# SCUT-CCNL/3DSIFT

Measured on AMD Instinct MI355X. Metric: Mvoxels/s end-to-end KpSiftAlgorithm on 512^3 fp32, higher is better.
Workload: dtype f32

## Files before the change

### 3dsift_amd/csrc/context.hip

```cpp
#include <float.h>
#include <math.h>
#include <stdlib.h>
#include <string.h>

#include <algorithm>
#include <atomic>
#include <mutex>
#include <thread>

#include "ctx_internal.h"

#pragma clang fp contract(off)

namespace s3d {

static thread_local std::string g_last_error;
void set_last_error(const std::string &s) { g_last_error = s; }

int set_device(int device) {
	int n = 0;
	if (hipGetDeviceCount(&n) != hipSuccess || n <= 0) {
		set_last_error("no HIP device visible: this library has no CPU fallback");
		return SIFT3D_ERR_NO_DEVICE;
	}
// ... 150 lines not shown
	c->gss.assign((size_t)c->noct * c->ng, Level());
	c->dog.assign((size_t)c->noct * c->nd, Level());
	for (int pyr = 0; pyr < 2; pyr++) {
		const int interval = pyr ? c->nd : c->ng;
		std::vector<Level> &P = pyr ? c->dog : c->gss;
		int nx = c->nx, ny = c->ny, nz = c->nz;
		float u = (float)(1 << c->octave_base);
		for (int o = 0; o < c->noct; o++) {
			for (int s = 0; s < interval; s++) {
				Level &L = P[(size_t)o * interval + s];
				L.nx = nx; L.ny = ny; L.nz = nz; L.unit = u;
				L.scale = level_scale(c->p, o + c->octave_base, s);
				if (c->slab) { L.bz = c->own1 - c->own0 + 2 * c->halo; L.zoff = c->own0 - c->halo; }
			}
			nx /= 2; ny /= 2; nz /= 2;
			u *= 2;
		}
	}
}

int upload_luts(sift3d_ctx *c, const std::vector<WinLut> &luts, std::vector<float> &pool) {
	if (pool.empty()) pool.push_back(-1.0f);
	if (c->d_luts) { S3D_HIP(hipFree(c->d_luts)); c->d_luts = nullptr; }
	if (c->d_lutpool) { S3D_HIP(hipFree(c->d_lutpool)); c->d_lutpool = nullptr; }
	S3D_HIP(hipMalloc(&c->d_luts, sizeof(WinLut) * luts.size()));
	S3D_HIP(hipMalloc(&c->d_lutpool, sizeof(float) * pool.size()));
	S3D_HIP(hipMemcpy(c->d_luts, luts.data(), sizeof(WinLut) * luts.size(), hipMemcpyHostToDevice));
	S3D_HIP(hipMemcpy(c->d_lutpool, pool.data(), sizeof(float) * pool.size(), hipMemcpyHostToDevice));
	return SIFT3D_OK;
}

std::vector<WinLut> blank_luts(const sift3d_ctx *c) {
	std::vector<WinLut> luts((size_t)std::max(1, c->noct + c->octave_base) * 8 * 2);
	for (auto &l : luts) { l.off = 0; l.len = 0; l.nin = -1; l.radius = 0; l.sigma = 0; l.fix_scale = 1.0f; l.wsum = 1.0f; l.list_off = -1; l.list_R = 0; }
	return luts;
}

static int build_luts(sift3d_ctx *c) {
	std::vector<WinLut> luts = blank_luts(c);
	std::vector<float> pool;
	for (int o = 0; o < c->noct; o++)
		for (int lv = 1; lv <= c->p.num_kp_levels && lv < 8; lv++) {
			const Level &D = c->dog[(size_t)o * c->nd + lv];
			const float u = D.unit, scale = D.scale;
			for (int which = 0; which < 2; which++) {
				float sigma, radius;
				if (which == 0) { sigma = 1.5f * scale; radius = sigma * 3.0f; }
				else { sigma = scale * 7.071067812f; radius = 2.0f * sigma; }
				if (!append_lut(pool, luts[((size_t)(o + c->octave_base) * 8 + lv) * 2 + which], which, sigma, radius, u, scale)) c->desc_lut_lds = false;
			}
		}
	return upload_luts(c, luts, pool);
}

static size_t al64(size_t n) { return (n + 63) & ~(size_t)63; }

size_t arena_floats_of(const sift3d_ctx *c) {
	size_t total = c->in_own ? 0 : al64(c->in.n());
	if (!c->slab) for (int o = 0; o < c->noct; o++) total += 2 * al64(c->gss[(size_t)o * c->ng].n());
	for (auto &L : c->gss) total += al64(L.n());
	for (auto &L : c->dog) total += al64(L.n());
	return total;
}

int create_common(sift3d_handle *out, const CreateCfg &cfg, const sift3d_params *params, int device) {
	*out = nullptr;
	if (cfg.nx <= 0 || cfg.ny <= 0 || cfg.nz <= 0) { set_last_error("bad dimensions"); return SIFT3D_ERR_ARG; }
// ... 785 lines not shown
```

### 3dsift_amd/csrc/kernels_orient.hip

```cpp
#include <float.h>

#include "sift3d_internal.h"

namespace s3d {

__device__ __forceinline__ float wave_sum(float v) {
#pragma unroll
	for (int o = 32; o > 0; o >>= 1) v = v + __shfl_xor(v, o, 64);
	return v;
}

__device__ __forceinline__ void win_bounds(float c, float rad, float u, int n, int &lo, int &hi) {
	int s = (int)floorf(c - __fdiv_rn(rad, u));
	lo = s > 1 ? s : 1;
	int e = (int)ceilf(c + __fdiv_rn(rad, u));
	hi = e < (n - 2) ? e : n - 2;
}

__device__ void eig_sym3(const double A[9], double w[3], double V[9]) {
	double a[9];
#pragma unroll
	for (int i = 0; i < 9; i++) { a[i] = A[i]; V[i] = (i % 4 == 0) ? 1.0 : 0.0; }
	for (int sweep = 0; sweep < 64; sweep++) {
		const double off = fabs(a[1]) + fabs(a[2]) + fabs(a[5]);
		const double diag = fabs(a[0]) + fabs(a[4]) + fabs(a[8]);
		if (off <= 1e-300 || off <= 1e-22 * diag) break;
#pragma unroll
		for (int pq = 0; pq < 3; pq++) {
			const int p = (pq == 2) ? 1 : 0, q = (pq == 0) ? 1 : 2;
			const double apq = a[3 * p + q];
			if (apq == 0.0) continue;
			const double theta = (a[4 * q] - a[4 * p]) / (2.0 * apq);
			const double t = (theta >= 0 ? 1.0 : -1.0) / (fabs(theta) + sqrt(theta * theta + 1.0));
// ... 71 lines not shown
	if ((double)fabsf(val[0] - val[1]) < DBL_EPSILON || (double)fabsf(val[0] - val[2]) < DBL_EPSILON ||
	    (double)fabsf(val[2] - val[1]) < DBL_EPSILON)
		return -2;

	const float d_norm = sqrtf(dot3f(w3, w3));
	float corner = FLT_MAX;
	for (int i = 2; i > 0; i--) {
		const float d = dot3f(vec[i], w3);
		const float q_norm = sqrtf(dot3f(vec[i], vec[i]));
		const float cos_ang = __fdiv_rn(d, d_norm * q_norm);
		const float a = fabsf(cos_ang);
		corner = corner < a ? corner : a;
		const float sgn = d > 0.0f ? 1.0f : -1.0f;
		vec[i][0] *= sgn; vec[i][1] *= sgn; vec[i][2] *= sgn;
	}
	nr = nr || fabsf(corner - corner_thresh) <= 1e-4f;
	if (near) *near = nr;
	if (corner < corner_thresh) return -3;
	if (near) *near = true;
	const float *v1 = vec[2], *v2 = vec[1];
	float vr[3];
	vr[0] = v1[1] * v2[2] - v1[2] * v2[1];
	vr[1] = v1[2] * v2[0] - v1[0] * v2[2];
	vr[2] = v1[0] * v2[1] - v1[1] * v2[0];
	kp.rot[0] = v1[0]; kp.rot[1] = v2[0]; kp.rot[2] = vr[0];
	kp.rot[3] = v1[1]; kp.rot[4] = v2[1]; kp.rot[5] = vr[1];
	kp.rot[6] = v1[2]; kp.rot[7] = v2[2]; kp.rot[8] = vr[2];
	return 1;
}

#ifndef S3D_ORI_UN
#define S3D_ORI_UN 2
#endif
constexpr int kTileW = 28, kTileH = 27;
constexpr int kTilePc = ((kTileW / 4) * kTileH + 63) / 64;
typedef float f4o __attribute__((ext_vector_type(4), aligned(4)));
constexpr int kOriLut = 256;

constexpr int kTermPitch = 68;
template <bool EXACT>
__global__ void __launch_bounds__(256) k_orient(DevKp *__restrict__ kps, int *__restrict__ codes, const unsigned *__restrict__ d_count, unsigned cap,
                                                const LevelRef *__restrict__ levels, const WinLut *__restrict__ luts,
                                                const float *__restrict__ lutpool, float max_eig, float corner, int part_rank,
                                                int part_world, const int *__restrict__ redo_list, const unsigned *__restrict__ redo_count) {
	__shared__ __attribute__((aligned(16))) float s_tile[4 * 3 * kTileW * kTileH];
	__shared__ float s_wlut[4 * kOriLut];
	__shared__ __attribute__((aligned(16))) float s_terms[EXACT ? 4 * 9 * kTermPitch : 4];
	const unsigned count = min(d_count[0], cap);
	const int lane = threadIdx.x & 63;
	const unsigned wave = blockIdx.x * (blockDim.x >> 6) + (threadIdx.x >> 6);
	const unsigned nwaves = gridDim.x * (blockDim.x >> 6);
	const unsigned pw = part_world > 1 ? (unsigned)part_world : 1u, pr = part_world > 1 ? (unsigned)part_rank : 0u;
	if (!EXACT && pw > 1)
		for (unsigned k = blockIdx.x * blockDim.x + threadIdx.x; k < count; k += gridDim.x * blockDim.x)
			if (k % pw != pr) { kps[k].code = 0; codes[k] = 0; }
	const unsigned owned = EXACT ? min(redo_count[0], cap) : (count > pr ? (count - pr + pw - 1) / pw : 0u);
	float *tb = &s_terms[EXACT ? (threadIdx.x >> 6) * 9 * kTermPitch : 0];
	for (unsigned j = wave; j < owned; j += nwaves) {
		const unsigned k = EXACT ? (unsigned)redo_list[j] : j * pw + pr;
		const int cxi = kps[k].x, cyi = kps[k].y, czi = kps[k].z;
		const int li = kps[k].octave * 8 + kps[k].level;
		const LevelRef L = levels[li];
		const WinLut lut = luts[li * 2 + 0];
		const float *__restrict__ wtab = lutpool + lut.off;
		const float u = L.unit, inv_u = __fdiv_rn(1.0f, u);
		int x0, x1, y0, y1, z0, z1;
		win_bounds((float)cxi, lut.radius, u, L.nx, x0, x1);
		win_bounds((float)cyi, lut.radius, u, L.ny, y0, y1);
		win_bounds((float)czi, lut.radius, u, L.nz, z0, z1);
		const int wx = x1 - x0 + 1, wy = y1 - y0 + 1;
		const int plane = (wx > 0 && wy > 0) ? wx * wy : 0;
		const float inv_wx = 1.0f / (float)(wx > 0 ? wx : 1);
		const size_t sy = (size_t)L.nx, sz = (size_t)L.nx * L.ny;
		const gfloat_p Ld = as_global(L.d);
		float t00 = 0.f, t01 = 0.f, t02 = 0.f, t11 = 0.f, t12 = 0.f, t22 = 0.f, g0 = 0.f, g1 = 0.f, g2 = 0.f;
		float chain = 0.f;
		auto emit = [&](bool ok, float c1p, float c1m, float c2p, float c2m, float c3p, float c3m, float ww, int nvalid) {
			float vx = 0.5f * (c1p - c1m);
			float vy = 0.5f * (c2p - c2m);
			float vz = 0.5f * (c3p - c3m);
			vx = vx * inv_u; vy = vy * inv_u; vz = vz * inv_u;
			if (!EXACT) {
				if (ok) {
					const float wx = vx * ww, wy = vy * ww, wz = vz * ww;
					t00 = __fmaf_rn(vx, wx, t00);
					t01 = __fmaf_rn(vx, wy, t01);
					t02 = __fmaf_rn(vx, wz, t02);
					t11 = __fmaf_rn(vy, wy, t11);
					t12 = __fmaf_rn(vy, wz, t12);
					t22 = __fmaf_rn(vz, wz, t22);
					g0 = g0 + wx; g1 = g1 + wy; g2 = g2 + wz;
				}
			} else {
				tb[0 * kTermPitch + lane] = ok ? vx * vx * ww : 0.0f;
				tb[1 * kTermPitch + lane] = ok ? vx * vy * ww : 0.0f;
				tb[2 * kTermPitch + lane] = ok ? vx * vz * ww : 0.0f;
				tb[3 * kTermPitch + lane] = ok ? vy * vy * ww : 0.0f;
				tb[4 * kTermPitch + lane] = ok ? vy * vz * ww : 0.0f;
				tb[5 * kTermPitch + lane] = ok ? vz * vz * ww : 0.0f;
				tb[6 * kTermPitch + lane] = ok ? vx * ww : 0.0f;
				tb[7 * kTermPitch + lane] = ok ? vy * ww : 0.0f;
				tb[8 * kTermPitch + lane] = ok ? vz * ww : 0.0f;
				__builtin_amdgcn_fence(__ATOMIC_RELEASE, "wavefront");
				__builtin_amdgcn_wave_barrier();
				__builtin_amdgcn_fence(__ATOMIC_ACQUIRE, "wavefront");
				if (lane < 9) {
					const float4 *row = reinterpret_cast<const float4 *>(tb + lane * kTermPitch);
#pragma unroll
					for (int h = 0; h < 2; h++) {
						if (h * 32 >= nvalid) break;
						float4 v[8];
#pragma unroll
						for (int i = 0; i < 8; i++) v[i] = row[h * 8 + i];
#pragma unroll
						for (int i = 0; i < 8; i++) { chain = chain + v[i].x; chain = chain + v[i].y; chain = chain + v[i].z; chain = chain + v[i].w; }
					}
				}
				__builtin_amdgcn_wave_barrier();
			}
		};
		const int tw = wx + 2, th = wy + 2;
		if (plane > 0 && z1 >= z0 && tw <= kTileW && th <= kTileH && lut.len <= kOriLut) {
			float *tile = &s_tile[(threadIdx.x >> 6) * 3 * kTileW * kTileH];
			float *wl = &s_wlut[(threadIdx.x >> 6) * kOriLut];
			for (int i = lane; i < lut.len && i < kOriLut; i += 64) wl[i] = wtab[i];
			const int npx = (tw + 3) >> 2;
			const int tnp = npx * th;
			const float inv_npx = 1.0f / (float)npx;
			int toff[kTilePc];
			int goff[kTilePc];
#pragma unroll
			for (int i = 0; i < kTilePc; i++) {
				const int idx = lane + 64 * i;
				const int ty = (int)(((float)idx + 0.5f) * inv_npx);
				const int px = idx - ty * npx;
				const bool ok = idx < tnp;
				toff[i] = ok ? ty * kTileW + 4 * px : -1;
				goff[i] = ok ? (x0 - 1 + 4 * px) + (int)sy * (y0 - 1 + ty) : (x0 - 1) + (int)sy * (y0 - 1);
			}
			const gfloat_p base = Ld - sz * (size_t)L.zoff;
			f4o pf[kTilePc];
			auto request = [&](int zp) {
				const gfloat_p pl = base + sz * (size_t)zp;
#pragma unroll
				for (int i = 0; i < kTilePc; i++) pf[i] = *reinterpret_cast<const f4o __attribute__((address_space(1))) *>(pl + goff[i]);
			};
			auto deposit = [&](int slot) {
				float *dstp = tile + slot * (kTileW * kTileH);
#pragma unroll
				for (int i = 0; i < kTilePc; i++)
					if (toff[i] >= 0) *reinterpret_cast<float4 *>(dstp + toff[i]) = make_float4(pf[i].x, pf[i].y, pf[i].z, pf[i].w);
			};
			request(z0 - 1); deposit(0);
			request(z0);     deposit(1);
			request(z0 + 1);
			int sm = 0, sc = 1, sp = 2;
			constexpr int kEL = 8;
			const unsigned *__restrict__ lst = reinterpret_cast<const unsigned *>(lutpool) + (lut.list_off >= 0 ? lut.list_off : 0);
			const int LR = lut.list_R;
			const unsigned *__restrict__ ent = lst + 2 * LR + 2;
			const bool use_list = lut.list_off >= 0 && (int)lst[LR + 1] - (int)lst[LR] <= 64 * kEL;
			const int ox = cxi - x0 - 128, oy = cyi - y0 - 128;
			unsigned En[kEL];
			int cntn = 0;
			auto fetch_entries = [&](int dzp) {
				const int pi = dzp + LR;
				const bool has = use_list && pi >= 0 && pi <= 2 * LR;
				const int e0 = has ? (int)lst[pi] : 0, e1 = has ? (int)lst[pi + 1] : 0;
				cntn = e1 - e0;
#pragma unroll
				for (int i = 0; i < kEL; i++) {
					const int idx = e0 + i * 64 + lane;
					En[i] = ent[idx < e1 ? idx : e0];
				}
			};
			fetch_entries(z0 - czi);
			for (int z = z0; z <= z1; z++) {
#if !defined(S3D_ODIAG) || !(S3D_ODIAG & 2)
				deposit(sp);
				request(min(z + 2, z1 + 1));
#endif
				__builtin_amdgcn_fence(__ATOMIC_RELEASE, "wavefront");
				__builtin_amdgcn_wave_barrier();
				__builtin_amdgcn_fence(__ATOMIC_ACQUIRE, "wavefront");
				const float *pm = tile + sm * (kTileW * kTileH), *pc = tile + sc * (kTileW * kTileH), *pp = tile + sp * (kTileW * kTileH);
				const int dz = z - czi;
				constexpr int kUn = S3D_ORI_UN;
#ifdef S3D_ODIAG
				if (S3D_ODIAG & 1) { } else
#endif
				if (use_list) {
					unsigned E[kEL];
#pragma unroll
					for (int i = 0; i < kEL; i++) E[i] = En[i];
					const int cnt = cntn;
					fetch_entries(dz + 1);
#pragma unroll
					for (int p0 = 0; p0 < kEL; p0 += kUn) {
						if (p0 * 64 >= cnt) break;
						float nb[kUn][6], w[kUn];
#pragma unroll
						for (int q = 0; q < kUn; q++) {
							const unsigned e = E[p0 + q];
							const int lx = (int)(e & 255u) + ox, ly = (int)((e >> 8) & 255u) + oy;
							const bool ok = (p0 + q) * 64 + lane < cnt && (unsigned)lx < (unsigned)wx && (unsigned)ly < (unsigned)wy;
							w[q] = ok ? wl[e >> 16] : -1.0f;
							const int o = ok ? __mul24(ly + 1, kTileW) + lx + 1 : kTileW + 1;
							nb[q][0] = pc[o + 1]; nb[q][1] = pc[o - 1]; nb[q][2] = pc[o + kTileW]; nb[q][3] = pc[o - kTileW];
							nb[q][4] = pp[o]; nb[q][5] = pm[o];
						}
#pragma unroll
						for (int q = 0; q < kUn; q++) {
							if (EXACT && (p0 + q) * 64 >= cnt) break;
							emit(!(w[q] < 0.0f), nb[q][0], nb[q][1], nb[q][2], nb[q][3], nb[q][4], nb[q][5], w[q], min(64, cnt - (p0 + q) * 64));
						}
					}
				} else if (EXACT) {
					for (int vb = 0; vb < plane; vb += 64) {
						const int v = vb + lane;
						const int ly = (int)(((float)v + 0.5f) * inv_wx);
						const int lx = v - ly * wx;
						const int dx = x0 + lx - cxi, dy = y0 + ly - cyi;
						const int n = dx * dx + dy * dy + dz * dz;
						const bool in = v < plane && n < lut.len;
						const float ww = in ? wl[n] : -1.0f;
						const int o = in ? __mul24(ly + 1, kTileW) + lx + 1 : kTileW + 1;
						emit(!(ww < 0.0f), pc[o + 1], pc[o - 1], pc[o + kTileW], pc[o - kTileW], pp[o], pm[o], ww, min(64, plane - vb));
					}
				} else
				for (int v0 = lane; v0 < plane; v0 += 64 * kUn) {
					float nb[kUn][6], w[kUn];
#pragma unroll
					for (int q = 0; q < kUn; q++) {
						const int v = v0 + 64 * q;
						const int ly = (int)(((float)v + 0.5f) * inv_wx);
						const int lx = v - ly * wx;
						const int dx = x0 + lx - cxi, dy = y0 + ly - cyi;
						const int n = dx * dx + dy * dy + dz * dz;
						const bool ok = v < plane && n < lut.len;
						w[q] = ok ? wl[n] : -1.0f;
						const int o = ok ? __mul24(ly + 1, kTileW) + lx + 1 : kTileW + 1;
						nb[q][0] = pc[o + 1]; nb[q][1] = pc[o - 1]; nb[q][2] = pc[o + kTileW]; nb[q][3] = pc[o - kTileW];
						nb[q][4] = pp[o]; nb[q][5] = pm[o];
					}
#pragma unroll
					for (int q = 0; q < kUn; q++)
						emit(!(w[q] < 0.0f), nb[q][0], nb[q][1], nb[q][2], nb[q][3], nb[q][4], nb[q][5], w[q], 64);
				}
				__builtin_amdgcn_wave_barrier();
				const int tmp = sm; sm = sc; sc = sp; sp = tmp;
			}
		} else
		for (int z = z0; z <= z1; z++) {
			const int dz = z - czi;
			for (int vb = 0; vb < plane; vb += 64) {
				const int v = vb + lane;
				const int ly = (int)(((float)v + 0.5f) * inv_wx);
				const int lx = v - ly * wx;
				const int x = x0 + lx, y = y0 + ly;
				const int dx = x - cxi, dy = y - cyi;
				const int n = dx * dx + dy * dy + dz * dz;
				const bool in = v < plane && n < lut.len;
				const float w = in ? wtab[n] : -1.0f;
				const bool ok = !(w < 0.0f);
				const gfloat_p c = ok ? Ld + (size_t)x + sy * (size_t)y + sz * (size_t)(z - L.zoff)
				                      : Ld + (size_t)cxi + sy * (size_t)cyi + sz * (size_t)(czi - L.zoff);
				emit(ok, c[1], c[-1], c[sy], *(c - sy), c[sz], *(c - sz), w, min(64, plane - vb));
			}
		}
// ... 9 lines not shown
			if (lane == 0) {
				kps[k].st[0] = T6[0]; kps[k].st[1] = T6[1]; kps[k].st[2] = T6[2]; kps[k].st[4] = T6[3]; kps[k].st[5] = T6[4]; kps[k].st[8] = T6[5];
				kps[k].win[0] = w3[0]; kps[k].win[1] = w3[1]; kps[k].win[2] = w3[2];
			}
		}
	}
}

__global__ void __launch_bounds__(64) k_orient_finish(DevKp *__restrict__ kps, int *__restrict__ codes, const unsigned *__restrict__ d_count,
                                                      unsigned cap, float max_eig, float corner, int part_rank, int part_world, int pass,
                                                      int *__restrict__ redo_list, unsigned *__restrict__ redo_count) {
	const unsigned count = min(d_count[0], cap);
	const unsigned pw = part_world > 1 ? (unsigned)part_world : 1u, pr = part_world > 1 ? (unsigned)part_rank : 0u;
	const unsigned owned = pass ? min(redo_count[0], cap) : (count > pr ? (count - pr + pw - 1) / pw : 0u);
	for (unsigned j = blockIdx.x * blockDim.x + threadIdx.x; j < owned; j += gridDim.x * blockDim.x) {
		const unsigned k = pass ? (unsigned)redo_list[j] : j * pw + pr;
		DevKp kp = kps[k];
		const float T6[6] = {kp.st[0], kp.st[1], kp.st[2], kp.st[4], kp.st[5], kp.st[8]};
		const float w3[3] = {kp.win[0], kp.win[1], kp.win[2]};
		bool near = false;
		kp.code = finish_orientation(kp, T6, w3, max_eig, corner, &near);
		kps[k] = kp;
		codes[k] = kp.code == 1 ? ((kp.level << 4) | 1) : kp.code;
		if (!pass && near) {
			const unsigned pos = atomicAdd(redo_count, 1u);
			if (pos < cap) redo_list[pos] = (int)k;
		}
	}
}

void launch_orient(DevKp *kps, int *codes, const unsigned *d_count, unsigned cap, const LevelRef *d_levels, const WinLut *d_luts,
                   const float *d_lutpool, float max_eig, float corner, int part_rank, int part_world, int *redo_list, unsigned *redo_count,
                   hipStream_t st) {
	static const int ori_grid = dev_tune_i("S3D_ORI_GRID", 256 * 32);
	(void)hipMemsetAsync(redo_count, 0, sizeof(unsigned), st);
	hipLaunchKernelGGL(k_orient<false>, dim3(ori_grid), dim3(256), 0, st, kps, codes, d_count, cap, d_levels, d_luts, d_lutpool, max_eig, corner,
	                   part_rank, part_world, (const int *)redo_list, (const unsigned *)redo_count);
	hipLaunchKernelGGL(k_orient_finish, dim3(256 * 8), dim3(64), 0, st, kps, codes, d_count, cap, max_eig, corner, part_rank, part_world, 0,
	                   redo_list, redo_count);
	hipLaunchKernelGGL(k_orient<true>, dim3(ori_grid), dim3(256), 0, st, kps, codes, d_count, cap, d_levels, d_luts, d_lutpool, max_eig, corner,
	                   part_rank, part_world, (const int *)redo_list, (const unsigned *)redo_count);
	hipLaunchKernelGGL(k_orient_finish, dim3(256 * 2), dim3(64), 0, st, kps, codes, d_count, cap, max_eig, corner, part_rank, part_world, 1,
	                   redo_list, redo_count);
}

static_assert(offsetof(DevKp, st) + sizeof(float) * 9 - offsetof(DevKp, win) == sizeof(float) * (kOrientWords - 1), "DevKp layout");

__global__ void __launch_bounds__(256) k_orient_pack(const DevKp *__restrict__ kps, const unsigned *__restrict__ d_count, unsigned cap,
                                                     int *__restrict__ dst, int part_rank, int part_world) {
	const unsigned count = min(d_count[0], cap);
	const unsigned total = count * (unsigned)kOrientWords;
	for (unsigned i = blockIdx.x * blockDim.x + threadIdx.x; i < total; i += gridDim.x * blockDim.x) {
		const unsigned k = i / kOrientWords, w = i - k * kOrientWords;
		int v = 0;
		if (part_world <= 1 || (int)(k % (unsigned)part_world) == part_rank)
			v = w == 0 ? kps[k].code : __float_as_int(kps[k].win[w - 1]);
		dst[i] = v;
	}
}

__global__ void __launch_bounds__(256) k_orient_unpack(DevKp *__restrict__ kps, int *__restrict__ codes, const unsigned *__restrict__ d_count,
                                                       unsigned cap, const int *__restrict__ src) {
	const unsigned count = min(d_count[0], cap);
	const unsigned total = count * (unsigned)kOrientWords;
	for (unsigned i = blockIdx.x * blockDim.x + threadIdx.x; i < total; i += gridDim.x * blockDim.x) {
		const unsigned k = i / kOrientWords, w = i - k * kOrientWords;
		const int v = src[i];
// ... 116 lines not shown
```

### 3dsift_amd/csrc/sift3d_internal.h

```cpp
#pragma once

#include <hip/hip_runtime.h>
#include <stdint.h>

#include <string>
#include <vector>

#include "../../include/sift3d_hip.h"
#include "../../include/sift3d_hip_test.h"

#pragma clang fp contract(off)

namespace s3d {

#ifndef S3D_MAX_HW
#define S3D_MAX_HW 64
#endif
constexpr int kMaxHW = S3D_MAX_HW;
constexpr int kMaxTaps = 2 * kMaxHW + 1;
constexpr int kDesc = SIFT3D_DESC_NUMEL;
constexpr int kFaces = 20;

struct Taps {
	int hw;
// ... 23 lines not shown
	size_t n() const { return (size_t)nx * ny * planes(); }
	ZRange zr(int zo0, int zo1) const { return ZRange{planes(), zoff, nz, zo0, zo1}; }
	ZRange zr_all() const { return ZRange{planes(), zoff, nz, 0, planes()}; }
};

struct DevKp {
	int x, y, z;
	int octave, level;
	float scale;
	int code;
	int slot;
	float win[3];
	float eigvalue[3];
	float eigvector[9];
	float rot[9];
	float st[9];
};

struct FaceConst {
	float e1[3], e2[3], t[3], q[3];
	float qe2;
	int idx[3];
	float centre[3];
};

struct WinLut {
	int off;
	int len;
	int nin;
	float radius;
	float sigma;
	float fix_scale;
	float wsum;
	int list_off, list_R;
};
constexpr int kMaxDescLut = 1536;

struct FaceSym {
	int face[32];
	int vert[32][3];
	int slot[32][3];
};

void launch_absmax(const float *src, size_t n, unsigned *d_max_bits, hipStream_t st, unsigned *d_nonfinite = nullptr);
void launch_scale_by_max(float *data, size_t n, const unsigned *d_max_bits, hipStream_t st);
void launch_dog_from_gss(const float *hi, const float *lo, float *dog, size_t n, hipStream_t st);
void launch_conv_axis(int axis, const float *src, float *dst, int nx, int ny, int nz, const Taps &t,
                      const float *prev, float *dog, unsigned *d_dogmax, hipStream_t st, bool exact = false);
struct MarchHalf { float *d = nullptr; int nx = 0, ny = 0, nz = 0; };
bool march_half_ok(int nx, int ny, const ZRange &zr);
bool march_applicable(int nx, int ny, int nzg, const Taps &t);
bool launch_march_level(const float *src, float *dst, float *dog, unsigned *dogmax, int nx, int ny, const ZRange &zr, const Taps &t,
                        hipStream_t st, int plan_slots = 0, int prio = 0, const MarchHalf *half = nullptr);
void launch_copy16(const float *src, float *dst, size_t nfloats, hipStream_t st);
constexpr int kCopySegs = 32, kMaxMergePtrs = 16;
struct CopySegs { const float *src[kCopySegs]; float *dst[kCopySegs]; size_t floats[kCopySegs]; int n = 0; };
struct MaxMerge { const float *in[kMaxMergePtrs]; float *out[kMaxMergePtrs]; int nin = 0, nout = 0, n = 0; };
void launch_copy_segments(const CopySegs &a, hipStream_t st);
void launch_max_merge(const MaxMerge &a, hipStream_t st);
constexpr int kSmallMaxOct = 4, kSmallMaxLv = 8;
struct SmallOct { float *g[kSmallMaxLv]; float *dog[kSmallMaxLv]; int nx, ny, nz; };
struct SmallArgs {
	SmallOct oct[kSmallMaxOct];
	int noct, ng, nd, seed;
	unsigned build_mask, dog_mask;
	unsigned *dogmax;
	int hwp;
	float w[kSmallMaxLv][9];
// ... 198 lines not shown
```

### 3dsift_amd/csrc/tables.hip

```cpp
#include <float.h>
#include <math.h>
#include <stdlib.h>
#include <string.h>

#include <algorithm>
#include <atomic>
#include <mutex>
#include <thread>

#include "ctx_internal.h"

#pragma clang fp contract(off)

namespace s3d {

bool build_taps(float sigma, Taps &t) {
	sigma = sigma > 0 ? sigma : 0;
	int hw = 1;
	if (sigma > 0) {
		hw = (int)ceil((double)sigma * 3.0);
		if (hw < 1) hw = 1;
	}
	if (hw > kMaxHW) return false;
	t.hw = hw;
// ... 99 lines not shown
}


bool append_lut(std::vector<float> &pool, WinLut &L, int which, float sigma, float radius, float u, float scale) {
	bool fits_lds = true;
	const float r2 = radius * radius, uu = u * u;
	const int len = (int)floor((double)r2 / (double)uu) + 2;
	L.off = (int)pool.size(); L.len = len; L.nin = -1; L.radius = radius; L.sigma = sigma; L.fix_scale = 1.0f; L.list_off = -1; L.list_R = 0;
	if (which == 1) {
		const double cw = 5.0 * (double)scale / (double)u, bound = (cw + 2.0) * (cw + 2.0) * (cw + 2.0) * 1.7321 * 1.001;
		int k = (int)floor(log2(2147483647.0 / bound));
		k = std::max(0, std::min(k, 29));
		L.fix_scale = (float)ldexp(1.0, k);
	}
	if (which == 1 && len > kMaxDescLut) fits_lds = false;
	for (int n = 0; n < len; n++) {
		const float sq = (float)n * uu;
		float w;
		if (!(sq > r2)) L.nin = n;
		if (sq > r2) w = -1.0f;
		else if (which == 0) w = expf((float)(-0.5 * (double)sq / (double)(sigma * sigma)));
		else w = expf(-0.5f * sq / (sigma * sigma)) * (0.5f / u);
		pool.push_back(w);
	}
	const int R = (int)floor(sqrt((double)std::max(L.nin, 0)));
	double ws = 0.0;
	for (int dz = -R; dz <= R; dz++)
		for (int dy = -R; dy <= R; dy++)
			for (int dx = -R; dx <= R; dx++) {
				const int n = dx * dx + dy * dy + dz * dz;
				if (n <= L.nin) ws += (double)pool[(size_t)L.off + n] * (which == 1 ? (double)u / 0.5 : 1.0);
			}
	L.wsum = (float)std::max(ws, 1.0);
	if (which == 0 && R <= 127 && L.nin < 65536) {
		std::vector<unsigned> words((size_t)2 * R + 2);
		for (int dz = -R; dz <= R; dz++) {
			words[(size_t)(dz + R)] = (unsigned)(words.size() - ((size_t)2 * R + 2));
			for (int dy = -R; dy <= R; dy++)
				for (int dx = -R; dx <= R; dx++) {
					const int n = dx * dx + dy * dy + dz * dz;
					if (n <= L.nin) words.push_back((unsigned)(dx + 128) | (unsigned)(dy + 128) << 8 | (unsigned)n << 16);
				}
		}
		words[(size_t)2 * R + 1] = (unsigned)(words.size() - ((size_t)2 * R + 2));
		L.list_off = (int)pool.size(); L.list_R = R;
		pool.resize(pool.size() + words.size());
		memcpy(pool.data() + L.list_off, words.data(), words.size() * sizeof(unsigned));
	}
	return fits_lds;
}

}
```

### 3dsift_amd/capi.py

```python
import ctypes as C
import os

import numpy as np

HERE = os.path.dirname(os.path.abspath(__file__))
LIB_PATH = os.environ.get("S3D_LIB") or os.path.join(HERE, "libsift3d_hip.so")
DESC = 768

KP_DTYPE = np.dtype(
    [
        ("x", "<f4"), ("y", "<f4"), ("z", "<f4"),
        ("scale", "<f4"),
        ("octave", "<i4"), ("level", "<i4"),
        ("rx", "<f4"), ("ry", "<f4"), ("rz", "<f4"),
        ("win", "<f4", (3,)),
        ("eigvalue", "<f4", (3,)),
        ("eigvector", "<f4", (9,)),
        ("Rotation", "<f4", (9,)),
        ("str_tensor", "<f4", (9,)),
    ]
)
assert KP_DTYPE.itemsize == 168

SYMBOLS = [
# ... 1 lines not shown
    "sift3d_stage_times", "sift3d_num_keypoints", "sift3d_get_keypoints", "sift3d_device_results",
    "sift3d_num_octaves", "sift3d_level_info", "sift3d_copy_level", "sift3d_copy_input", "sift3d_num_extrema",
    "sift3d_get_extrema", "sift3d_get_orientation_codes", "sift3d_gaussian_smooth", "sift3d_downsample", "sift3d_dog_sub", "sift3d_conv_axis",
    "sift3d_orient_keypoint", "sift3d_describe_keypoint", "sift3d_match",
    "sift3d_match_handles",
    "sift3d_default_detect_options", "sift3d_set_detect_options", "sift3d_get_detect_options", "sift3d_get_refined",
    "sift3d_default_ransac_options", "sift3d_fit_affine", "sift3d_fit_affine_local",
    "sift3d_default_icgn_options", "sift3d_icgn_init_from_fits", "sift3d_icgn",
    "sift3d_bspline_prefilter", "sift3d_icgn_bspline",
    "sift3d_icgn2_init_from_icgn", "sift3d_icgn2", "sift3d_strain_input_from_icgn2",
    "sift3d_default_search_options", "sift3d_zncc_search", "sift3d_icgn_init_from_search",
    "sift3d_default_strain_options", "sift3d_strain_input_from_icgn", "sift3d_strain",
    "sift3d_default_validate_options", "sift3d_validate_input_from_icgn", "sift3d_validate_input_from_icgn2", "sift3d_validate_displacements",
    "sift3d_validate_keep", "sift3d_icgn_init_from_validation", "sift3d_validate_stage_capacity",
    "sift3d_device_count", "sift3d_error_string", "sift3d_last_error",
    "sift3d_slab_min_halo", "sift3d_slab_arena_floats", "sift3d_slab_create", "sift3d_slab_buffer", "sift3d_slab_upload",
    "sift3d_slab_input_absmax", "sift3d_slab_input_scale", "sift3d_slab_level", "sift3d_slab_level_hw", "sift3d_slab_halo_planes",
    "sift3d_slab_sync", "sift3d_slab_get_dogmax", "sift3d_slab_set_dogmax", "sift3d_slab_detect", "sift3d_slab_describe",
    "sift3d_slab_decimate", "sift3d_slab_admits", "sift3d_slab_set_ghost", "sift3d_slab_min_halo_ghost", "sift3d_create_seeded", "sift3d_seed_upload", "sift3d_set_describe_partition",
    "sift3d_export_device", "sift3d_import_descriptors_device", "sift3d_run_partial_orientation",
    "sift3d_export_orientation_device", "sift3d_import_orientation_device", "sift3d_run_describe",
    "sift3d_set_stream", "sift3d_slab_export_dogmax_device", "sift3d_slab_import_dogmax_device", "sift3d_slab_decimate_async",
    "sift3d_slab_set_desc_partial", "sift3d_slab_min_halo_partial", "sift3d_slab_record_bytes", "sift3d_slab_desc_reach", "sift3d_slab_orient",
    "sift3d_slab_export_records", "sift3d_slab_describe_partial", "sift3d_slab_describe_finish", "sift3d_slab_orient_launch",
    "sift3d_slab_orient_count",
    "sift3d_slab_keypoints_launch", "sift3d_slab_keypoints_count", "sift3d_slab_describe_finish_launch", "sift3d_slab_describe_finish_count",
    "sift3d_seed_buffer", "sift3d_sharded_plan", "sift3d_slab_describe_launch", "sift3d_sharded_traffic",
    "sift3d_sharded_create", "sift3d_sharded_create_ex", "sift3d_sharded_run", "sift3d_sharded_num_keypoints", "sift3d_sharded_get_keypoints", "sift3d_sharded_info",
    "sift3d_sharded_error", "sift3d_sharded_destroy",
    "sift3d_test_hook", "sift3d_debug_counters", "sift3d_debug_face_lookup", "sift3d_match_times", "sift3d_debug_copy_bandwidth",
    "sift3d_match_warmup", "sift3d_test_staging_slice", "sift3d_test_slab_plan", "sift3d_test_sharded_time_rank",
]
HOOKS = {"dog_eager": 0, "glast_eager": 1, "det_serial": 2, "separable": 3, "desc_nocache": 4, "match_nodma": 5, "one_stream": 6,
         "desc_mass_shift": 7, "list_cap": 8, "peer_copy": 9, "desc_nosplit": 10, "march_tiles": 11, "desc_exact_cells": 12, "lazy_generic": 13, "sharded_fail_rank": 14}
ORIENT_WORDS = 34
SHARDED_PARTIAL_WINDOWS = 1
SHARDED_WHOLE_WINDOWS = 2
SHARDED_COPY_TRANSPORT = 4
SHARDED_GHOST_OCTAVE0 = 8


class Params(C.Structure):
    _fields_ = [("num_kp_levels", C.c_int), ("sigma_default", C.c_float), ("sigma_n_default", C.c_float),
                ("peak_thresh", C.c_float), ("max_eig_thres", C.c_float), ("corner_thresh", C.c_float)]


class DetectOptions(C.Structure):
    _fields_ = [("neighbours", C.c_int), ("refine", C.c_int), ("max_offset", C.c_float), ("contrast_thresh", C.c_float),
                ("edge_ratio", C.c_float), ("reserved", C.c_int * 3)]


assert C.sizeof(DetectOptions) == 32

REFINED_DTYPE = np.dtype([("rx", "<f4"), ("ry", "<f4"), ("rz", "<f4"), ("scale", "<f4"), ("offset", "<f4", (4,)), ("contrast", "<f4")])
assert REFINED_DTYPE.itemsize == 36


class RansacOptions(C.Structure):
    _fields_ = [("iterations", C.c_int), ("inlier_thresh", C.c_float), ("seed", C.c_uint), ("refine", C.c_int), ("min_det", C.c_float),
                ("reserved", C.c_int * 3)]


assert C.sizeof(RansacOptions) == 32

FIT_DTYPE = np.dtype([("A", "<f8", (12,)), ("hyp", "<f8", (12,)), ("status", "<i4"), ("candidates", "<i4"), ("best_hypothesis", "<i4"),
                      ("best_count", "<i4"), ("inliers", "<i4"), ("rms", "<f4"), ("reserved", "<i4", (2,))])
assert FIT_DTYPE.itemsize == 224
# ... 1222 lines not shown
```

Before: 19860.

## Repack orientation offset list with precomputed tile byte offsets and fast whole-window path

Repacks each orientation window list entry so it carries a precomputed LDS byte offset, packed dx/dy and a pre-scaled weight index, and pads the list so per-slice fetches need no bounds clamping. The kernel reads per-slice start offsets through readlane instead of global loads and uses byte-offset addressing. When the window is not clipped at the volume edge it takes a specialised path that skips the per-entry bounds checks. It also pins the wave index as uniform, sets a minimum-occupancy launch bound, and adds a host-side layout validation that aborts on violation. The cost is extra register pressure from the occupancy hint and more host table work.

New measurement: 19810. Within noise of the previous version (-0.2%).

```diff
diff --git a/3dsift_amd/csrc/context.hip b/3dsift_amd/csrc/context.hip
--- a/3dsift_amd/csrc/context.hip
+++ b/3dsift_amd/csrc/context.hip
@@ -206,7 +206,7 @@
 
 std::vector<WinLut> blank_luts(const sift3d_ctx *c) {
 	std::vector<WinLut> luts((size_t)std::max(1, c->noct + c->octave_base) * 8 * 2);
-	for (auto &l : luts) { l.off = 0; l.len = 0; l.nin = -1; l.radius = 0; l.sigma = 0; l.fix_scale = 1.0f; l.wsum = 1.0f; l.list_off = -1; l.list_R = 0; }
+	for (auto &l : luts) { l.off = 0; l.len = 0; l.nin = -1; l.radius = 0; l.sigma = 0; l.fix_scale = 1.0f; l.wsum = 1.0f; l.list_off = -1; l.list_R = 0; l.list_W = -1; }
 	return luts;
 }
 
diff --git a/3dsift_amd/csrc/kernels_orient.hip b/3dsift_amd/csrc/kernels_orient.hip
--- a/3dsift_amd/csrc/kernels_orient.hip
+++ b/3dsift_amd/csrc/kernels_orient.hip
@@ -1,4 +1,6 @@
 #include <float.h>
+
+#include <type_traits>
 
 #include "sift3d_internal.h"
 
@@ -136,14 +138,13 @@
 #ifndef S3D_ORI_UN
 #define S3D_ORI_UN 2
 #endif
-constexpr int kTileW = 28, kTileH = 27;
+constexpr int kTileW = kOriTileW, kTileH = kOriTileH, kOriLut = kOriLutLen, kEL = kOriListSlots;
 constexpr int kTilePc = ((kTileW / 4) * kTileH + 63) / 64;
 typedef float f4o __attribute__((ext_vector_type(4), aligned(4)));
-constexpr int kOriLut = 256;
 
 constexpr int kTermPitch = 68;
 template <bool EXACT>
-__global__ void __launch_bounds__(256) k_orient(DevKp *__restrict__ kps, int *__restrict__ codes, const unsigned *__restrict__ d_count, unsigned cap,
+__global__ void __launch_bounds__(256, EXACT ? 3 : 4) k_orient(DevKp *__restrict__ kps, int *__restrict__ codes, const unsigned *__restrict__ d_count, unsigned cap,
                                                 const LevelRef *__restrict__ levels, const WinLut *__restrict__ luts,
                                                 const float *__restrict__ lutpool, float max_eig, float corner, int part_rank,
                                                 int part_world, const int *__restrict__ redo_list, const unsigned *__restrict__ redo_count) {
@@ -152,14 +153,15 @@
 	__shared__ __attribute__((aligned(16))) float s_terms[EXACT ? 4 * 9 * kTermPitch : 4];
 	const unsigned count = min(d_count[0], cap);
 	const int lane = threadIdx.x & 63;
-	const unsigned wave = blockIdx.x * (blockDim.x >> 6) + (threadIdx.x >> 6);
+	const unsigned wv = (unsigned)__builtin_amdgcn_readfirstlane((int)(threadIdx.x >> 6));
+	const unsigned wave = blockIdx.x * (blockDim.x >> 6) + wv;
 	const unsigned nwaves = gridDim.x * (blockDim.x >> 6);
 	const unsigned pw = part_world > 1 ? (unsigned)part_world : 1u, pr = part_world > 1 ? (unsigned)part_rank : 0u;
 	if (!EXACT && pw > 1)
 		for (unsigned k = blockIdx.x * blockDim.x + threadIdx.x; k < count; k += gridDim.x * blockDim.x)
 			if (k % pw != pr) { kps[k].code = 0; codes[k] = 0; }
 	const unsigned owned = EXACT ? min(redo_count[0], cap) : (count > pr ? (count - pr + pw - 1) / pw : 0u);
-	float *tb = &s_terms[EXACT ? (threadIdx.x >> 6) * 9 * kTermPitch : 0];
+	float *tb = &s_terms[EXACT ? wv * 9 * kTermPitch : 0];
 	for (unsigned j = wave; j < owned; j += nwaves) {
 		const unsigned k = EXACT ? (unsigned)redo_list[j] : j * pw + pr;
 		const int cxi = kps[k].x, cyi = kps[k].y, czi = kps[k].z;
@@ -225,14 +227,14 @@
 		};
 		const int tw = wx + 2, th = wy + 2;
 		if (plane > 0 && z1 >= z0 && tw <= kTileW && th <= kTileH && lut.len <= kOriLut) {
-			float *tile = &s_tile[(threadIdx.x >> 6) * 3 * kTileW * kTileH];
-			float *wl = &s_wlut[(threadIdx.x >> 6) * kOriLut];
+			float *tile = &s_tile[wv * 3 * kTileW * kTileH];
+			float *wl = &s_wlut[wv * kOriLut];
 			for (int i = lane; i < lut.len && i < kOriLut; i += 64) wl[i] = wtab[i];
 			const int npx = (tw + 3) >> 2;
 			const int tnp = npx * th;
 			const float inv_npx = 1.0f / (float)npx;
 			int toff[kTilePc];
-			int goff[kTilePc];
+			unsigned goff[kTilePc];
 #pragma unroll
 			for (int i = 0; i < kTilePc; i++) {
 				const int idx = lane + 64 * i;
@@ -240,12 +242,13 @@
 				const int px = idx - ty * npx;
 				const bool ok = idx < tnp;
 				toff[i] = ok ? ty * kTileW + 4 * px : -1;
-				goff[i] = ok ? (x0 - 1 + 4 * px) + (int)sy * (y0 - 1 + ty) : (x0 - 1) + (int)sy * (y0 - 1);
+				goff[i] = 4u * (unsigned)(ok ? (x0 - 1 + 4 * px) + (int)sy * (y0 - 1 + ty) : (x0 - 1) + (int)sy * (y0 - 1));
 			}
 			const gfloat_p base = Ld - sz * (size_t)L.zoff;
 			f4o pf[kTilePc];
+			typedef const char __attribute__((address_space(1))) *gbyte_p;
 			auto request = [&](int zp) {
-				const gfloat_p pl = base + sz * (size_t)zp;
+				const gbyte_p pl = reinterpret_cast<gbyte_p>(base + sz * (size_t)zp);
 #pragma unroll
 				for (int i = 0; i < kTilePc; i++) pf[i] = *reinterpret_cast<const f4o __attribute__((address_space(1))) *>(pl + goff[i]);
 			};
@@ -259,26 +262,28 @@
 			request(z0);     deposit(1);
 			request(z0 + 1);
 			int sm = 0, sc = 1, sp = 2;
-			constexpr int kEL = 8;
 			const unsigned *__restrict__ lst = reinterpret_cast<const unsigned *>(lutpool) + (lut.list_off >= 0 ? lut.list_off : 0);
 			const int LR = lut.list_R;
 			const unsigned *__restrict__ ent = lst + 2 * LR + 2;
 			const bool use_list = lut.list_off >= 0 && (int)lst[LR + 1] - (int)lst[LR] <= 64 * kEL;
-			const int ox = cxi - x0 - 128, oy = cyi - y0 - 128;
+			const bool whole = use_list && lut.list_W >= 0 && cxi - x0 == lut.list_W && x1 - cxi == lut.list_W && cyi - y0 == lut.list_W && y1 - cyi == lut.list_W;
+			const int ox = cxi - x0 - 16, oy = cyi - y0 - 16;
+			const unsigned starts = use_list && lane < 2 * LR + 2 ? lst[lane] : 0u;
 			unsigned En[kEL];
+#pragma unroll
+			for (int i = 0; i < kEL; i++) En[i] = 0u;
 			int cntn = 0;
 			auto fetch_entries = [&](int dzp) {
 				const int pi = dzp + LR;
-				const bool has = use_list && pi >= 0 && pi <= 2 * LR;
-				const int e0 = has ? (int)lst[pi] : 0, e1 = has ? (int)lst[pi + 1] : 0;
-				cntn = e1 - e0;
-#pragma unroll
-				for (int i = 0; i < kEL; i++) {
-					const int idx = e0 + i * 64 + lane;
-					En[i] = ent[idx < e1 ? idx : e0];
-				}
+				const bool has = pi >= 0 && pi <= 2 * LR;
+				const unsigned e0 = has ? (unsigned)__builtin_amdgcn_readlane((int)starts, has ? pi : 0) : 0u;
+				const unsigned e1 = has ? (unsigned)__builtin_amdgcn_readlane((int)starts, has ? pi + 1 : 0) : 0u;
+				cntn = (int)(e1 - e0);
+				const unsigned *__restrict__ pl = ent + e0;
+#pragma unroll
+				for (int i = 0; i < kEL; i++) En[i] = pl[(unsigned)lane + 64u * i];
 			};
-			fetch_entries(z0 - czi);
+			if (use_list) fetch_entries(z0 - czi);
 			for (int z = z0; z <= z1; z++) {
 #if !defined(S3D_ODIAG) || !(S3D_ODIAG & 2)
 				deposit(sp);
@@ -299,26 +304,50 @@
 					for (int i = 0; i < kEL; i++) E[i] = En[i];
 					const int cnt = cntn;
 					fetch_entries(dz + 1);
-#pragma unroll
-					for (int p0 = 0; p0 < kEL; p0 += kUn) {
-						if (p0 * 64 >= cnt) break;
-						float nb[kUn][6], w[kUn];
-#pragma unroll
-						for (int q = 0; q < kUn; q++) {
-							const unsigned e = E[p0 + q];
-							const int lx = (int)(e & 255u) + ox, ly = (int)((e >> 8) & 255u) + oy;
-							const bool ok = (p0 + q) * 64 + lane < cnt && (unsigned)lx < (unsigned)wx && (unsigned)ly < (unsigned)wy;
-							w[q] = ok ? wl[e >> 16] : -1.0f;
-							const int o = ok ? __mul24(ly + 1, kTileW) + lx + 1 : kTileW + 1;
-							nb[q][0] = pc[o + 1]; nb[q][1] = pc[o - 1]; nb[q][2] = pc[o + kTileW]; nb[q][3] = pc[o - kTileW];
-							nb[q][4] = pp[o]; nb[q][5] = pm[o];
+					const int left = cnt - lane;
+					const unsigned wlast = 4u * (unsigned)(lut.len - 1);
+					auto passes = [&](auto whole_c, auto nq_c, const unsigned *Ep, int p0) {
+						constexpr bool kWhole = decltype(whole_c)::value;
+						constexpr int nq = decltype(nq_c)::value;
+						float nb[nq][6], w[nq];
+#pragma unroll
+						for (int q = 0; q < nq; q++) {
+							const unsigned e = Ep[q];
+							unsigned ob, wb;
+							if (kWhole) {
+								wb = (p0 + q) * 64 < left ? e >> 22 : wlast;
+								ob = e & 0xffcu;
+							} else {
+								const int lx = (int)((e >> 12) & 31u) + ox, ly = (int)((e >> 17) & 31u) + oy;
+								const bool ok = (p0 + q) * 64 < left && (unsigned)lx < (unsigned)wx && (unsigned)ly < (unsigned)wy;
+								wb = ok ? e >> 22 : wlast;
+								ob = 4u * (unsigned)(ok ? __mul24(ly + 1, kTileW) + lx + 1 : kTileW + 1);
+							}
+							w[q] = *reinterpret_cast<const float *>(reinterpret_cast<const char *>(wl) + wb);
+							const float *c = reinterpret_cast<const float *>(reinterpret_cast<const char *>(pc) + ob);
+							nb[q][0] = c[1]; nb[q][1] = c[-1]; nb[q][2] = c[kTileW]; nb[q][3] = c[-kTileW];
+							nb[q][4] = *reinterpret_cast<const float *>(reinterpret_cast<const char *>(pp) + ob);
+							nb[q][5] = *reinterpret_cast<const float *>(reinterpret_cast<const char *>(pm) + ob);
 						}
 #pragma unroll
-						for (int q = 0; q < kUn; q++) {
+						for (int q = 0; q < nq; q++) {
 							if (EXACT && (p0 + q) * 64 >= cnt) break;
 							emit(!(w[q] < 0.0f), nb[q][0], nb[q][1], nb[q][2], nb[q][3], nb[q][4], nb[q][5], w[q], min(64, cnt - (p0 + q) * 64));
 						}
-					}
+					};
+					const int ng = cnt > 64 ? (cnt - 65) / (64 * kUn) + 1 : 0;
+					unsigned tail = E[0];
+#pragma unroll
+					for (int i = kUn; i < kEL; i += kUn) tail = ng >= i / kUn ? E[i] : tail;
+					auto walk = [&](auto whole_c) {
+#pragma unroll
+						for (int p0 = 0; p0 < kEL; p0 += kUn) {
+							if (p0 / kUn >= ng) break;
+							passes(whole_c, std::integral_constant<int, kUn>(), &E[p0], p0);
+						}
+						if (cnt > ng * kUn * 64) passes(whole_c, std::integral_constant<int, 1>(), &tail, ng * kUn);
+					};
+					if (whole) walk(std::true_type()); else walk(std::false_type());
 				} else if (EXACT) {
 					for (int vb = 0; vb < plane; vb += 64) {
 						const int v = vb + lane;
diff --git a/3dsift_amd/csrc/sift3d_internal.h b/3dsift_amd/csrc/sift3d_internal.h
--- a/3dsift_amd/csrc/sift3d_internal.h
+++ b/3dsift_amd/csrc/sift3d_internal.h
@@ -79,8 +79,11 @@
 	float sigma;
 	float fix_scale;
 	float wsum;
-	int list_off, list_R;
-};
+	int list_off, list_R, list_W;
+};
+constexpr int kOriTileW = 28, kOriTileH = 27;
+constexpr int kOriLutLen = 256;
+constexpr int kOriListSlots = 8;
 constexpr int kMaxDescLut = 1536;
 
 struct FaceSym {
diff --git a/3dsift_amd/csrc/tables.hip b/3dsift_amd/csrc/tables.hip
--- a/3dsift_amd/csrc/tables.hip
+++ b/3dsift_amd/csrc/tables.hip
@@ -155,17 +155,41 @@
 				if (n <= L.nin) ws += (double)pool[(size_t)L.off + n] * (which == 1 ? (double)u / 0.5 : 1.0);
 			}
 	L.wsum = (float)std::max(ws, 1.0);
-	if (which == 0 && R <= 127 && L.nin < 65536) {
-		std::vector<unsigned> words((size_t)2 * R + 2);
+	L.list_W = -1;
+	if (which == 0 && len <= kOriLutLen && R <= 15) {
+		const int W = (int)ceilf(radius / u);
+		const bool fits = W >= R && 2 * W + 3 <= kOriTileW && 2 * W + 3 <= kOriTileH;
+		if (fits) L.list_W = W;
+		auto entry = [&](int dx, int dy, int n) {
+			const unsigned tile = fits ? (unsigned)((dy + W + 1) * kOriTileW + dx + W + 1) : 0u;
+			return 4u * tile | (unsigned)(dx + 16) << 12 | (unsigned)(dy + 16) << 17 | 4u * (unsigned)n << 22;
+		};
+		const size_t head = (size_t)2 * R + 2;
+		std::vector<unsigned> words(head);
 		for (int dz = -R; dz <= R; dz++) {
-			words[(size_t)(dz + R)] = (unsigned)(words.size() - ((size_t)2 * R + 2));
+			words[(size_t)(dz + R)] = (unsigned)(words.size() - head);
 			for (int dy = -R; dy <= R; dy++)
 				for (int dx = -R; dx <= R; dx++) {
 					const int n = dx * dx + dy * dy + dz * dz;
-					if (n <= L.nin) words.push_back((unsigned)(dx + 128) | (unsigned)(dy + 128) << 8 | (unsigned)n << 16);
+					if (n <= L.nin) words.push_back(entry(dx, dy, n));
 				}
 		}
-		words[(size_t)2 * R + 1] = (unsigned)(words.size() - ((size_t)2 * R + 2));
+		const size_t nent = words.size() - head;
+		words[head - 1] = (unsigned)nent;
+		words.resize(words.size() + (size_t)kOriListSlots * 64, entry(0, 0, 0));
+		bool good = words.size() == head + nent + (size_t)kOriListSlots * 64 && pool[(size_t)L.off + len - 1] == -1.0f;
+		for (size_t p = 0; p + 1 < head && good; p++) good = words[p] <= words[p + 1] && (size_t)words[p] + kOriListSlots * 64 <= words.size() - head;
+		for (size_t i = head; i < words.size() && good; i++) {
+			const unsigned e = words[i];
+			const int dx = (int)(e >> 12 & 31u) - 16, dy = (int)(e >> 17 & 31u) - 16, n = (int)(e >> 24), tile = (int)(e & 0xfffu) / 4;
+			good = (e & 3u) == 0 && (e >> 22 & 3u) == 0 && n <= L.nin && n < len - 1 && abs(dx) <= R && abs(dy) <= R &&
+			       (i < head + nent || (dx == 0 && dy == 0 && n == 0)) &&
+			       (fits ? tile == (dy + W + 1) * kOriTileW + dx + W + 1 && tile - kOriTileW >= 1 && tile + kOriTileW < kOriTileW * kOriTileH : tile == 0);
+		}
+		if (!good) {
+			fprintf(stderr, "append_lut: the orientation list of radius %g / unit %g breaks its layout or padding rule (WinLut)\n", (double)radius, (double)u);
+			abort();
+		}
 		L.list_off = (int)pool.size(); L.list_R = R;
 		pool.resize(pool.size() + words.size());
 		memcpy(pool.data() + L.list_off, words.data(), words.size() * sizeof(unsigned));
```

## Skip out-of-sphere tile loads and stream entry lists in orientation kernel

Applied to the files above, without the earlier changes.

Orientation kernel now marks wave-uniform values (keypoint coords, window bounds, wave index) with readfirstlane so they stay in scalar registers. It precomputes a per-chunk minimum squared distance and skips global loads of tile chunks that lie outside the spherical window for the current plane when the entry-list path is used. Entry-list loading is restructured: plane start offsets come from a lane register via readlane, and next-plane entries are loaded slot by slot interleaved with processing instead of a full double-buffered prefetch, with an explicit waitcnt. A test hook for overriding the grid size is also added. Skipped chunks leave stale data in shared tile cells, which is safe only if those cells are never read for in-window voxels.

After: 19290 before, 19810 after (median of 6 runs). +2.7%, better.

```diff
diff --git a/3dsift_amd/capi.py b/3dsift_amd/capi.py
--- a/3dsift_amd/capi.py
+++ b/3dsift_amd/capi.py
@@ -57,7 +57,8 @@
     "sift3d_match_warmup", "sift3d_test_staging_slice", "sift3d_test_slab_plan", "sift3d_test_sharded_time_rank",
 ]
 HOOKS = {"dog_eager": 0, "glast_eager": 1, "det_serial": 2, "separable": 3, "desc_nocache": 4, "match_nodma": 5, "one_stream": 6,
-         "desc_mass_shift": 7, "list_cap": 8, "peer_copy": 9, "desc_nosplit": 10, "march_tiles": 11, "desc_exact_cells": 12, "lazy_generic": 13, "sharded_fail_rank": 14}
+         "desc_mass_shift": 7, "list_cap": 8, "peer_copy": 9, "desc_nosplit": 10, "march_tiles": 11, "desc_exact_cells": 12, "lazy_generic": 13, "sharded_fail_rank": 14,
+         "ori_grid": 15}
 ORIENT_WORDS = 34
 SHARDED_PARTIAL_WINDOWS = 1
 SHARDED_WHOLE_WINDOWS = 2
diff --git a/3dsift_amd/csrc/kernels_orient.hip b/3dsift_amd/csrc/kernels_orient.hip
--- a/3dsift_amd/csrc/kernels_orient.hip
+++ b/3dsift_amd/csrc/kernels_orient.hip
@@ -152,18 +152,19 @@
 	__shared__ __attribute__((aligned(16))) float s_terms[EXACT ? 4 * 9 * kTermPitch : 4];
 	const unsigned count = min(d_count[0], cap);
 	const int lane = threadIdx.x & 63;
-	const unsigned wave = blockIdx.x * (blockDim.x >> 6) + (threadIdx.x >> 6);
+	const unsigned wib = (unsigned)__builtin_amdgcn_readfirstlane((int)(threadIdx.x >> 6));
+	const unsigned wave = blockIdx.x * (blockDim.x >> 6) + wib;
 	const unsigned nwaves = gridDim.x * (blockDim.x >> 6);
 	const unsigned pw = part_world > 1 ? (unsigned)part_world : 1u, pr = part_world > 1 ? (unsigned)part_rank : 0u;
 	if (!EXACT && pw > 1)
 		for (unsigned k = blockIdx.x * blockDim.x + threadIdx.x; k < count; k += gridDim.x * blockDim.x)
 			if (k % pw != pr) { kps[k].code = 0; codes[k] = 0; }
 	const unsigned owned = EXACT ? min(redo_count[0], cap) : (count > pr ? (count - pr + pw - 1) / pw : 0u);
-	float *tb = &s_terms[EXACT ? (threadIdx.x >> 6) * 9 * kTermPitch : 0];
+	float *tb = &s_terms[EXACT ? wib * 9 * kTermPitch : 0];
 	for (unsigned j = wave; j < owned; j += nwaves) {
-		const unsigned k = EXACT ? (unsigned)redo_list[j] : j * pw + pr;
-		const int cxi = kps[k].x, cyi = kps[k].y, czi = kps[k].z;
-		const int li = kps[k].octave * 8 + kps[k].level;
+		const unsigned k = EXACT ? (unsigned)__builtin_amdgcn_readfirstlane(redo_list[j]) : j * pw + pr;
+		const int cxi = __builtin_amdgcn_readfirstlane(kps[k].x), cyi = __builtin_amdgcn_readfirstlane(kps[k].y), czi = __builtin_amdgcn_readfirstlane(kps[k].z);
+		const int li = __builtin_amdgcn_readfirstlane(kps[k].octave * 8 + kps[k].level);
 		const LevelRef L = levels[li];
 		const WinLut lut = luts[li * 2 + 0];
 		const float *__restrict__ wtab = lutpool + lut.off;
@@ -172,6 +173,9 @@
 		win_bounds((float)cxi, lut.radius, u, L.nx, x0, x1);
 		win_bounds((float)cyi, lut.radius, u, L.ny, y0, y1);
 		win_bounds((float)czi, lut.radius, u, L.nz, z0, z1);
+		x0 = __builtin_amdgcn_readfirstlane(x0); x1 = __builtin_amdgcn_readfirstlane(x1);
+		y0 = __builtin_amdgcn_readfirstlane(y0); y1 = __builtin_amdgcn_readfirstlane(y1);
+		z0 = __builtin_amdgcn_readfirstlane(z0); z1 = __builtin_amdgcn_readfirstlane(z1);
 		const int wx = x1 - x0 + 1, wy = y1 - y0 + 1;
 		const int plane = (wx > 0 && wy > 0) ? wx * wy : 0;
 		const float inv_wx = 1.0f / (float)(wx > 0 ? wx : 1);
@@ -225,14 +229,20 @@
 		};
 		const int tw = wx + 2, th = wy + 2;
 		if (plane > 0 && z1 >= z0 && tw <= kTileW && th <= kTileH && lut.len <= kOriLut) {
-			float *tile = &s_tile[(threadIdx.x >> 6) * 3 * kTileW * kTileH];
-			float *wl = &s_wlut[(threadIdx.x >> 6) * kOriLut];
+			float *tile = &s_tile[wib * 3 * kTileW * kTileH];
+			float *wl = &s_wlut[wib * kOriLut];
+			const int LR = lut.list_R;
+			const bool has_list = lut.list_off >= 0 && 2 * LR + 2 <= 64;
+			const unsigned *__restrict__ lst = reinterpret_cast<const unsigned *>(lutpool) + (has_list ? lut.list_off : 0);
+			const int starts = has_list && lane < 2 * LR + 2 ? (int)lst[lane] : 0;
 			for (int i = lane; i < lut.len && i < kOriLut; i += 64) wl[i] = wtab[i];
 			const int npx = (tw + 3) >> 2;
 			const int tnp = npx * th;
 			const float inv_npx = 1.0f / (float)npx;
 			int toff[kTilePc];
 			int goff[kTilePc];
+			int pd2[kTilePc];
+			const int cxt = cxi - x0 + 1, cyt = cyi - y0 + 1;
 #pragma unroll
 			for (int i = 0; i < kTilePc; i++) {
 				const int idx = lane + 64 * i;
@@ -241,13 +251,18 @@
 				const bool ok = idx < tnp;
 				toff[i] = ok ? ty * kTileW + 4 * px : -1;
 				goff[i] = ok ? (x0 - 1 + 4 * px) + (int)sy * (y0 - 1 + ty) : (x0 - 1) + (int)sy * (y0 - 1);
+				const int ax = max(max(4 * px - cxt, cxt - (4 * px + 3)) - 1, 0), ay = max(abs(ty - cyt) - 1, 0);
+				pd2[i] = ok ? ax * ax + ay * ay : 0x7fffffff;
 			}
 			const gfloat_p base = Ld - sz * (size_t)L.zoff;
-			f4o pf[kTilePc];
-			auto request = [&](int zp) {
+			f4o pf[kTilePc] = {};
+			auto request = [&](int zp, bool part) {
 				const gfloat_p pl = base + sz * (size_t)zp;
-#pragma unroll
-				for (int i = 0; i < kTilePc; i++) pf[i] = *reinterpret_cast<const f4o __attribute__((address_space(1))) *>(pl + goff[i]);
+				const int az = max(abs(zp - czi) - 1, 0);
+				const int lim = part ? lut.nin - az * az : 0x7ffffffe;
+#pragma unroll
+				for (int i = 0; i < kTilePc; i++)
+					if (pd2[i] <= lim) pf[i] = *reinterpret_cast<const f4o __attribute__((address_space(1))) *>(pl + goff[i]);
 			};
 			auto deposit = [&](int slot) {
 				float *dstp = tile + slot * (kTileW * kTileH);
@@ -255,34 +270,36 @@
 				for (int i = 0; i < kTilePc; i++)
 					if (toff[i] >= 0) *reinterpret_cast<float4 *>(dstp + toff[i]) = make_float4(pf[i].x, pf[i].y, pf[i].z, pf[i].w);
 			};
-			request(z0 - 1); deposit(0);
-			request(z0);     deposit(1);
-			request(z0 + 1);
+			request(z0 - 1, false); deposit(0);
+			request(z0, false);     deposit(1);
+			request(z0 + 1, false);
 			int sm = 0, sc = 1, sp = 2;
 			constexpr int kEL = 8;
-			const unsigned *__restrict__ lst = reinterpret_cast<const unsigned *>(lutpool) + (lut.list_off >= 0 ? lut.list_off : 0);
-			const int LR = lut.list_R;
 			const unsigned *__restrict__ ent = lst + 2 * LR + 2;
-			const bool use_list = lut.list_off >= 0 && (int)lst[LR + 1] - (int)lst[LR] <= 64 * kEL;
+			const bool use_list = has_list && __builtin_amdgcn_readlane(starts, has_list ? LR + 1 : 0) - __builtin_amdgcn_readlane(starts, has_list ? LR : 0) <= 64 * kEL;
 			const int ox = cxi - x0 - 128, oy = cyi - y0 - 128;
-			unsigned En[kEL];
-			int cntn = 0;
-			auto fetch_entries = [&](int dzp) {
+			unsigned E[kEL] = {0u, 0u, 0u, 0u, 0u, 0u, 0u, 0u};
+			int cnt = 0, cntn = 0;
+			const unsigned *__restrict__ pen = ent;
+			auto plane_entries = [&](int dzp) {
 				const int pi = dzp + LR;
 				const bool has = use_list && pi >= 0 && pi <= 2 * LR;
-				const int e0 = has ? (int)lst[pi] : 0, e1 = has ? (int)lst[pi + 1] : 0;
+				const int e0 = has ? __builtin_amdgcn_readlane(starts, pi) : 0, e1 = has ? __builtin_amdgcn_readlane(starts, pi + 1) : 0;
 				cntn = e1 - e0;
-#pragma unroll
-				for (int i = 0; i < kEL; i++) {
-					const int idx = e0 + i * 64 + lane;
-					En[i] = ent[idx < e1 ? idx : e0];
-				}
+				pen = ent + e0;
 			};
-			fetch_entries(z0 - czi);
+			auto load_slot = [&](int i) { E[i] = pen[min((unsigned)(i * 64 + lane), (unsigned)(cntn - 1))]; };
+			plane_entries(z0 - czi);
+#pragma unroll
+			for (int i = 0; i < kEL; i++) {
+				if (i * 64 >= cntn) break;
+				load_slot(i);
+			}
 			for (int z = z0; z <= z1; z++) {
+				__builtin_amdgcn_s_waitcnt(0x0F70);
 #if !defined(S3D_ODIAG) || !(S3D_ODIAG & 2)
 				deposit(sp);
-				request(min(z + 2, z1 + 1));
+				request(min(z + 2, z1 + 1), use_list);
 #endif
 				__builtin_amdgcn_fence(__ATOMIC_RELEASE, "wavefront");
 				__builtin_amdgcn_wave_barrier();
@@ -294,36 +311,26 @@
 				if (S3D_ODIAG & 1) { } else
 #endif
 				if (use_list) {
-					unsigned E[kEL];
-#pragma unroll
-					for (int i = 0; i < kEL; i++) E[i] = En[i];
-					const int cnt = cntn;
-					fetch_entries(dz + 1);
-#pragma unroll
-					for (int p0 = 0; p0 < kEL; p0 += kUn) {
-						if (p0 * 64 >= cnt) break;
-						float nb[kUn][6], w[kUn];
-#pragma unroll
-						for (int q = 0; q < kUn; q++) {
-							const unsigned e = E[p0 + q];
+					cnt = cntn;
+					plane_entries(dz + 1);
+#pragma unroll
+					for (int i = 0; i < kEL; i++) {
+						if (i * 64 >= cnt && i * 64 >= cntn) break;
+						if (i * 64 < cnt) {
+							const unsigned e = E[i];
 							const int lx = (int)(e & 255u) + ox, ly = (int)((e >> 8) & 255u) + oy;
-							const bool ok = (p0 + q) * 64 + lane < cnt && (unsigned)lx < (unsigned)wx && (unsigned)ly < (unsigned)wy;
-							w[q] = ok ? wl[e >> 16] : -1.0f;
+							const bool ok = i * 64 + lane < cnt && (unsigned)lx < (unsigned)wx && (unsigned)ly < (unsigned)wy;
+							const float w = ok ? wl[e >> 16] : -1.0f;
 							const int o = ok ? __mul24(ly + 1, kTileW) + lx + 1 : kTileW + 1;
-							nb[q][0] = pc[o + 1]; nb[q][1] = pc[o - 1]; nb[q][2] = pc[o + kTileW]; nb[q][3] = pc[o - kTileW];
-							nb[q][4] = pp[o]; nb[q][5] = pm[o];
+							emit(ok, pc[o + 1], pc[o - 1], pc[o + kTileW], pc[o - kTileW], pp[o], pm[o], w, min(64, cnt - i * 64));
 						}
-#pragma unroll
-						for (int q = 0; q < kUn; q++) {
-							if (EXACT && (p0 + q) * 64 >= cnt) break;
-							emit(!(w[q] < 0.0f), nb[q][0], nb[q][1], nb[q][2], nb[q][3], nb[q][4], nb[q][5], w[q], min(64, cnt - (p0 + q) * 64));
-						}
+						if (i * 64 < cntn) load_slot(i);
 					}
 				} else if (EXACT) {
 					for (int vb = 0; vb < plane; vb += 64) {
 						const int v = vb + lane;
 						const int ly = (int)(((float)v + 0.5f) * inv_wx);
-						const int lx = v - ly * wx;
+						const int lx = v - __mul24(ly, wx);
 						const int dx = x0 + lx - cxi, dy = y0 + ly - cyi;
 						const int n = dx * dx + dy * dy + dz * dz;
 						const bool in = v < plane && n < lut.len;
@@ -332,13 +339,13 @@
 						emit(!(ww < 0.0f), pc[o + 1], pc[o - 1], pc[o + kTileW], pc[o - kTileW], pp[o], pm[o], ww, min(64, plane - vb));
 					}
 				} else
-				for (int v0 = lane; v0 < plane; v0 += 64 * kUn) {
+				for (int vb = 0; vb < plane; vb += 64 * kUn) {
 					float nb[kUn][6], w[kUn];
 #pragma unroll
 					for (int q = 0; q < kUn; q++) {
-						const int v = v0 + 64 * q;
+						const int v = vb + lane + 64 * q;
 						const int ly = (int)(((float)v + 0.5f) * inv_wx);
-						const int lx = v - ly * wx;
+						const int lx = v - __mul24(ly, wx);
 						const int dx = x0 + lx - cxi, dy = y0 + ly - cyi;
 						const int n = dx * dx + dy * dy + dz * dz;
 						const bool ok = v < plane && n < lut.len;
@@ -414,7 +421,8 @@
 void launch_orient(DevKp *kps, int *codes, const unsigned *d_count, unsigned cap, const LevelRef *d_levels, const WinLut *d_luts,
                    const float *d_lutpool, float max_eig, float corner, int part_rank, int part_world, int *redo_list, unsigned *redo_count,
                    hipStream_t st) {
-	static const int ori_grid = dev_tune_i("S3D_ORI_GRID", 256 * 32);
+	static const int dflt_grid = dev_tune_i("S3D_ORI_GRID", 256 * 32);
+	const int ori_grid = hook(SIFT3D_HOOK_ORI_GRID) > 0 ? hook(SIFT3D_HOOK_ORI_GRID) : dflt_grid;
 	(void)hipMemsetAsync(redo_count, 0, sizeof(unsigned), st);
 	hipLaunchKernelGGL(k_orient<false>, dim3(ori_grid), dim3(256), 0, st, kps, codes, d_count, cap, d_levels, d_luts, d_lutpool, max_eig, corner,
 	                   part_rank, part_world, (const int *)redo_list, (const unsigned *)redo_count);
```
